# ysymyth/3D-SDN

Hardware: AMD Instinct MI355X
Metric: rendered-objects/sec (FFD decode + transform + silhouette/normal/depth @384, fwd+bwd) (higher is better)
Workload: dtype f32

## Files before the change

### 3d-sdn_amd/csrc/fast_ffd.hip

```cpp
#include "sdn_common.h"

namespace sdn {

constexpr int NCOEF_MAX = 512;

__global__ __launch_bounds__(256) void k_ffd_fwd(const float* __restrict__ Bt, const float* __restrict__ P,
                                                  const int32_t* __restrict__ cls, int vmax, int ncoef,
                                                  float* __restrict__ out)
{
    __shared__ float Ps[3 * NCOEF_MAX];
    const int b = blockIdx.y;
    for (int t = threadIdx.x; t < 3 * ncoef; t += 256) Ps[t] = P[(size_t)b * 3 * ncoef + t];
    __syncthreads();
    const int v = blockIdx.x * 256 + threadIdx.x;
    if (v >= vmax) return;
    const float* bt = Bt + (size_t)cls[b] * ncoef * vmax + v;
    float x = 0.f, y = 0.f, z = 0.f;
#pragma unroll 8
    for (int j = 0; j < ncoef; j++) {
        const float w = bt[(size_t)j * vmax];
        x += Ps[j] * w;
        y += Ps[ncoef + j] * w;
        z += Ps[2 * ncoef + j] * w;
    }
// ... 3 lines not shown
    o[2] = z;
}

constexpr int FFD_BWD_THREADS = 1024, FFD_JB = 4;
__global__ __launch_bounds__(FFD_BWD_THREADS) void k_ffd_bwd(const float* __restrict__ Bt, const int32_t* __restrict__ cls,
                                                              const float* __restrict__ g, int vmax, int ncoef,
                                                              float* __restrict__ grad_P)
{
    constexpr int NW = FFD_BWD_THREADS / 64;
    __shared__ float red[FFD_JB][3][NW];
    const int b = blockIdx.y, j0 = blockIdx.x * FFD_JB;
    const float* bt = Bt + ((size_t)cls[b] * ncoef + j0) * vmax;
    const float* gb = g + (size_t)b * vmax * 3;
    float s[FFD_JB][3];
#pragma unroll
    for (int u = 0; u < FFD_JB; u++) s[u][0] = s[u][1] = s[u][2] = 0.f;
#pragma unroll 2
    for (int v = threadIdx.x; v < vmax; v += FFD_BWD_THREADS) {
        const float g0 = gb[3 * v + 0], g1 = gb[3 * v + 1], g2 = gb[3 * v + 2];
#pragma unroll
        for (int u = 0; u < FFD_JB; u++) {
            const float w = (j0 + u < ncoef) ? bt[(size_t)u * vmax + v] : 0.f;
            s[u][0] += g0 * w;
            s[u][1] += g1 * w;
            s[u][2] += g2 * w;
        }
    }
#pragma unroll
    for (int u = 0; u < FFD_JB; u++) {
#pragma unroll
        for (int o = 32; o > 0; o >>= 1) {
            s[u][0] += __shfl_xor(s[u][0], o, 64);
            s[u][1] += __shfl_xor(s[u][1], o, 64);
            s[u][2] += __shfl_xor(s[u][2], o, 64);
        }
        if ((threadIdx.x & 63) == 0) {
            red[u][0][threadIdx.x >> 6] = s[u][0];
            red[u][1][threadIdx.x >> 6] = s[u][1];
            red[u][2][threadIdx.x >> 6] = s[u][2];
        }
    }
    __syncthreads();
    if (threadIdx.x < 3 * FFD_JB) {
        const int u = threadIdx.x / 3, d = threadIdx.x % 3;
        if (j0 + u < ncoef) {
            float t = 0.f;
#pragma unroll
            for (int w = 0; w < NW; w++) t += red[u][d][w];
            grad_P[((size_t)b * 3 + d) * ncoef + j0 + u] = t;
        }
    }
}

__global__ __launch_bounds__(256) void k_ffd_coefficients(const float* __restrict__ x, const float* __restrict__ M,
                                                          const float* __restrict__ base, int m, int transpose,
                                                          float* __restrict__ out)
{
    extern __shared__ float xrow[];
    float* part = xrow + m;
    const int i = blockIdx.y;
    for (int k = threadIdx.x; k < m; k += 256) xrow[k] = x[(size_t)i * m + k];
    __syncthreads();
    const int jj = threadIdx.x & 63, kq = threadIdx.x >> 6;
    const int j = blockIdx.x * 64 + jj;
    const int per = (m + 3) / 4, k0 = kq * per, k1 = min(m, k0 + per);
    float acc = 0.0f;
    if (j < m) {
        if (transpose) {
            const float* row = M + (size_t)j * m;
#pragma unroll 8
            for (int k = k0; k < k1; k++) acc = fmaf(xrow[k], row[k], acc);
        } else {
#pragma unroll 8
            for (int k = k0; k < k1; k++) acc = fmaf(xrow[k], M[(size_t)k * m + j], acc);
        }
    }
    part[kq * 64 + jj] = acc;
    __syncthreads();
    if (kq == 0 && j < m)
        out[(size_t)i * m + j] = (base ? base[j] : 0.0f) + ((part[jj] + part[64 + jj]) + (part[128 + jj] + part[192 + jj]));
}

}

using namespace sdn;

SDN_API int sdn_ffd_coefficients(const float* x, const float* M, const float* base, int n, int m, int transpose, float* out,
                                 sdnStream stream)
{
    if (!x || !M || !out || n <= 0 || m <= 0 || m > 12288)
        return fail(SDN_EINVAL, "sdn_ffd_coefficients: bad arguments (m <= 12288)");
    hipLaunchKernelGGL(k_ffd_coefficients, dim3(cdiv(m, 64), n), dim3(256), (size_t)(m + 256) * sizeof(float), (hipStream_t)stream,
                       x, M, base, m, transpose, out);
    return check_launch("k_ffd_coefficients");
}

SDN_API int sdn_ffd_decode(const float* Bt, const float* P, const int32_t* cls, int n, int vmax, int ncoef, float* out,
                           sdnStream stream)
{
    if (!Bt || !P || !cls || !out || n <= 0 || vmax <= 0 || ncoef <= 0 || ncoef > NCOEF_MAX)
        return fail(SDN_EINVAL, "sdn_ffd_decode: bad arguments (ncoef <= %d)", NCOEF_MAX);
    hipLaunchKernelGGL(k_ffd_fwd, dim3(cdiv(vmax, 256), n), dim3(256), 0, (hipStream_t)stream, Bt, P, cls, vmax, ncoef,
                       out);
    return check_launch("k_ffd_fwd");
}

SDN_API int sdn_ffd_decode_bwd(const float* Bt, const int32_t* cls, const float* grad_out, int n, int vmax, int ncoef,
                               float* grad_P, sdnStream stream)
{
    if (!Bt || !cls || !grad_out || !grad_P || n <= 0 || vmax <= 0 || ncoef <= 0 || ncoef > NCOEF_MAX)
        return fail(SDN_EINVAL, "sdn_ffd_decode_bwd: bad arguments");
    hipLaunchKernelGGL(k_ffd_bwd, dim3(cdiv(ncoef, FFD_JB), n), dim3(FFD_BWD_THREADS), 0, (hipStream_t)stream, Bt, cls, grad_out, vmax, ncoef,
                       grad_P);
    return check_launch("k_ffd_bwd");
}
```

### 3d-sdn_amd/csrc/raster_bwd.hip

```cpp
#include "raster_math.h"
#include "sdn_common.h"

namespace sdn {

#ifndef SDN_EDGE_CHUNK
#define SDN_EDGE_CHUNK 8
#endif
constexpr int CHUNK = SDN_EDGE_CHUNK;
static_assert(CHUNK == 4 || CHUNK == 8, "k_edge_scan_sil / k_chunk_sum are written for 4 or 8");

struct BwdParams {
    const float* faces;
    const float* textures;
    const float* face_inv;
    const int32_t* face_index_map;
    const float* weight_map;
    const float* depth_map;
    const float* rgb_map;
    const float* g_rgb_out;
    const float* g_alpha_out;
    const float* g_depth_out;
    float* grad_faces;
    float* grad_textures;
    uint32_t* visible;
// ... 187 lines not shown
            if (M.fidx(x, y) != fn) continue;
            float diff_grad = 0.0f;
            if (use_alpha) diff_grad = diff_grad + (1.0f - alpha_out) * M.g_alpha(x, y);
            if (use_rgb) {
#pragma unroll
                for (int k = 0; k < 3; k++) diff_grad = diff_grad + (M.rgb(x, y, k) - rgb_out[k]) * M.g_rgb(x, y, k);
            }
            if (diff_grad <= 0) continue;
            if (nz1) acc0 -= diff_grad / edge_dist(w.p[0][0], w.p[1][0], den1, d1, d1_cross, is_f, P.eps);
            if (nz0) acc1 -= diff_grad / edge_dist(w.p[0][0], w.p[1][0], den0, d1, d1_cross, is_f, P.eps);
        }
    }
}

__global__ __launch_bounds__(256) void k_mark_visible(const int32_t* __restrict__ face_index_map, long npx, int S,
                                                       int nf, uint32_t* __restrict__ visible)
{
    const long i = (long)blockIdx.x * 256 + threadIdx.x;
    if (i >= npx) return;
    const int fn = face_index_map[i];
    if (fn >= 0) visible[(i / ((long)S * S)) * nf + fn] = 1u;
}

__global__ __launch_bounds__(256) void k_hmap(const BwdParams P, float* __restrict__ hmapT)
{
    __shared__ float tile[32][33];
    const int S = P.S, b = blockIdx.z;
    const MapReader M(P, b);
    const int x = blockIdx.x * 32 + (threadIdx.x & 31);
#pragma unroll
    for (int r = 0; r < 4; r++) {
        const int ly = (threadIdx.x >> 5) + 8 * r, y = blockIdx.y * 32 + ly;
        float h = 0.0f;
        if (x < S && y < S) {
            const int fn = M.fidx(x, y);
            if (fn < 0) {
                const float t = (0.0f - 1.0f) * M.g_alpha(x, y);
                h = t > 0.0f ? t : 0.0f;
            } else {
                P.visible[(size_t)b * P.nf + fn] = 1u;
            }
        }
        tile[ly][threadIdx.x & 31] = h;
    }
    __syncthreads();
    const int yt = blockIdx.y * 32 + (threadIdx.x & 31);
#pragma unroll
    for (int r = 0; r < 4; r++) {
        const int lx = (threadIdx.x >> 5) + 8 * r, xt = blockIdx.x * 32 + lx;
        if (xt < S && yt < S) hmapT[((size_t)b * S + xt) * S + yt] = tile[threadIdx.x & 31][lx];
    }
}

__global__ __launch_bounds__(256) void k_compact_rows(const BwdParams P, const float* __restrict__ mapsT,
                                                      size_t rows_per_map, int S, uint16_t* __restrict__ cnt,
                                                      uint16_t* __restrict__ pos, float* __restrict__ val)
{
    const int lane = threadIdx.x & 63;
    const size_t row = (size_t)blockIdx.x * 4 + (threadIdx.x >> 6);
    if (row >= 2 * rows_per_map) return;
    const bool image_row = row < rows_per_map;
    const float* src = mapsT + (image_row ? 0 : row - rows_per_map) * S;
    const int yb = (int)(row / (size_t)S), yy = (int)(row % (size_t)S);
    const MapReader M(P, image_row ? yb : 0);
    auto h_at = [&](const int x) {
        float h = 0.0f;
        if (M.fidx(x, yy) < 0) {
            const float t = (0.0f - 1.0f) * M.g_alpha(x, yy);
            h = t > 0.0f ? t : 0.0f;
        }
        return h;
    };
    uint16_t* c = cnt + row * (S + 1);
    int base = 0;
    for (int x0 = 0; x0 < S; x0 += 128) {
        const int x = x0 + 2 * lane;
        float h0 = 0.0f, h1 = 0.0f;
        if (image_row) {
            if (x < S) h0 = h_at(x);
            if (x + 1 < S) h1 = h_at(x + 1);
        } else if (x + 1 < S && ((S & 1) == 0)) {
            const float2 v = *reinterpret_cast<const float2*>(src + x);
            h0 = v.x;
            h1 = v.y;
        } else {
            if (x < S) h0 = src[x];
            if (x + 1 < S) h1 = src[x + 1];
        }
        const bool nz0 = h0 > 0.0f, nz1 = h1 > 0.0f;
        const unsigned long long m0 = __ballot(nz0), m1 = __ballot(nz1);
        const unsigned long long below = (1ull << lane) - 1ull;
        const int i0 = base + __popcll(m0 & below) + __popcll(m1 & below);
        const int i1 = i0 + (nz0 ? 1 : 0);
        if (x < S) {
            c[x] = (uint16_t)i0;
            if (nz0) {
                pos[row * S + i0] = (uint16_t)x;
                val[row * S + i0] = h0;
            }
        }
        if (x + 1 < S) {
            c[x + 1] = (uint16_t)i1;
            if (nz1) {
                pos[row * S + i1] = (uint16_t)(x + 1);
                val[row * S + i1] = h1;
            }
        }
        base += __popcll(m0) + __popcll(m1);
    }
    if (lane == 0) c[S] = (uint16_t)base;
}

constexpr int PLAN_THREADS = 1024;
__global__ __launch_bounds__(PLAN_THREADS) void k_edge_plan(const BwdParams P)
{
    const long i = (long)blockIdx.x * PLAN_THREADS + threadIdx.x;
    const long total = (long)P.bs * P.nf;
    if (P.sink.grad_verts) {
        const long n = (long)P.bs * P.sink.nv * 3;
        for (long k = i; k < n; k += (long)gridDim.x * PLAN_THREADS) P.sink.grad_verts[k] = 0.0f;
    }
    const int lane = threadIdx.x & 63;
    int from[6], cnt[6];
    uint32_t nchunks = 0;
    bool contributes = false;
    if (i < total) {
        const bool active = (P.flags & (SDN_ALPHA | SDN_RGB)) != 0;
        if (active && P.visible[i] != 0u) {
            float face[9];
#pragma unroll
            for (int k = 0; k < 9; k++) face[k] = P.faces[i * 9 + k];
            if (!is_backface(face)) {
                const float is_f = (float)P.S;
#pragma unroll
                for (int e = 0; e < 6; e++) {
                    const EdgeWalk w = edge_walk(face, e >> 1, e & 1, is_f);
                    from[e] = w.d0_from;
                    cnt[e] = max(w.d0_to - w.d0_from + 1, 0);
                    nchunks += (uint32_t)((cnt[e] + CHUNK - 1) / CHUNK);
                }
                contributes = nchunks != 0;
            }
        }
    }
    __shared__ uint32_t wave_sum[PLAN_THREADS / 64];
    __shared__ uint32_t block_base;
    uint32_t incl = nchunks;
#pragma unroll
    for (int d = 1; d < 64; d <<= 1) {
        const uint32_t o = __shfl_up(incl, d, 64);
        if (lane >= d) incl += o;
    }
    const int wave = threadIdx.x >> 6;
    if (lane == 63) wave_sum[wave] = incl;
    __syncthreads();
    if (threadIdx.x == 0) {
        uint32_t tot = 0;
        for (int w = 0; w < PLAN_THREADS / 64; w++) tot += wave_sum[w];
        block_base = tot ? atomicAdd(P.counter, tot) : 0u;
    }
    __syncthreads();
    uint32_t wave_base = block_base;
    for (int w = 0; w < wave; w++) wave_base += wave_sum[w];
    if (i >= total) return;
    if (!contributes) {
        P.chunk_base[i] = -2;
        return;
    }
    const uint32_t base = wave_base + incl - nchunks;
    if (base + nchunks > P.cap) {
        P.chunk_base[i] = -1;
        for (uint32_t c = base; c < P.cap; c++) P.chunk_desc[c] = make_uint4(0xffffffffu, 0xffffffffu, 0u, 0u);
        return;
    }
    P.chunk_base[i] = (int32_t)base;
    uint32_t c = base;
#pragma unroll
    for (int e = 0; e < 6; e++) {
        for (int s = 0; s < cnt[e]; s += CHUNK)
            P.chunk_desc[c++] = make_uint4((uint32_t)i, (uint32_t)e, (uint32_t)(from[e] + s),
                                           (uint32_t)min(CHUNK, cnt[e] - s));
    }
}

__global__ __launch_bounds__(256) void k_edge_scan(const BwdParams P)
{
    const int lane = threadIdx.x & 63;
    const uint32_t wave = (blockIdx.x * 256u + threadIdx.x) >> 6;
    const uint32_t nwaves = (gridDim.x * 256u) >> 6;
    const uint32_t nchunks = min(*P.counter, P.cap);
    const bool use_alpha = (P.flags & SDN_ALPHA) != 0;
    const bool use_rgb = (P.flags & SDN_RGB) != 0;
    const float is_f = (float)P.S;
    for (uint32_t c = wave; c < nchunks; c += nwaves) {
        const uint4 d = P.chunk_desc[c];
        if (d.x >= (uint32_t)((long)P.bs * P.nf)) {
            if (lane == 0) P.chunk_out[c] = make_float2(0.f, 0.f);
            continue;
        }
        const long i = d.x;
        const int bn = (int)(i / P.nf), fn = (int)(i % P.nf);
        float face[9];
#pragma unroll
        for (int k = 0; k < 9; k++) face[k] = P.faces[i * 9 + k];
        const int axis = (int)(d.y & 1u);
        const EdgeWalk w = edge_walk(face, (int)(d.y >> 1), axis, is_f);
        const MapReader M(P, bn);
        float acc0 = 0.f, acc1 = 0.f;
        for (int s = 0; s < (int)d.w; s++)
            edge_pixel(P, M, w, fn, axis, (int)d.z + s, use_alpha, use_rgb, lane, 64, acc0, acc1);
#pragma unroll
        for (int o = 32; o > 0; o >>= 1) {
            acc0 += __shfl_xor(acc0, o, 64);
            acc1 += __shfl_xor(acc1, o, 64);
        }
        if (lane == 0) P.chunk_out[c] = make_float2(acc0, acc1);
    }
}

#ifndef SDN_LAB_IN_LANE_MAX
#define SDN_LAB_IN_LANE_MAX 32
#endif
constexpr int IN_LANE_MAX = SDN_LAB_IN_LANE_MAX;
#ifndef SDN_LAB_COOP_MAX_WALKS
#define SDN_LAB_COOP_MAX_WALKS 32
#endif
constexpr int COOP_MAX_WALKS = SDN_LAB_COOP_MAX_WALKS;

__global__ __launch_bounds__(256) void k_edge_scan_sil(const BwdParams P)
{
    const int lane = threadIdx.x & 63;
    const uint32_t wave = (blockIdx.x * 256u + threadIdx.x) >> 6;
    const uint32_t nwaves = (gridDim.x * 256u) >> 6;
    const uint32_t nchunks = min(*P.counter, P.cap);
    const int S = P.S;
// ... 507 lines not shown
        return fail(SDN_EINVAL, "rasterize_bwd_core: the vertex sink takes a silhouette-only pass");
    if ((flags & SDN_RGB) && (!rgb_map || !textures))
        return fail(SDN_EINVAL, "sdn_rasterize_bwd: rgb gradients need rgb_map and textures");
    if ((flags & SDN_AA) && (S & 1)) return fail(SDN_EINVAL, "sdn_rasterize_bwd: SDN_AA needs an even internal size");
    size_t off[14], need;
    uint32_t cap;
    bwd_layout(bs, nf, S, off, cap, need);
    if (!workspace || workspace_bytes < need)
        return fail(SDN_ENOMEM, "sdn_rasterize_bwd: workspace %zu < %zu bytes", workspace_bytes, need);
    hipStream_t st = (hipStream_t)stream;
    BwdParams P;
    P.faces = faces;
    P.textures = textures;
    P.face_inv = face_inv;
    P.face_index_map = face_index_map;
    P.weight_map = weight_map;
    P.depth_map = depth_map;
    P.rgb_map = rgb_map;
    P.g_rgb_out = (flags & SDN_RGB) ? g_rgb_out : nullptr;
    P.g_alpha_out = (flags & SDN_ALPHA) ? g_alpha_out : nullptr;
    P.g_depth_out = (flags & SDN_DEPTH) ? g_depth_out : nullptr;
    P.grad_faces = grad_faces;
    P.grad_textures = grad_textures;
    char* ws = (char*)workspace;
    P.counter = (uint32_t*)(ws + off[0]);
    P.visible = (uint32_t*)(ws + off[1]);
    P.chunk_base = (int32_t*)(ws + off[2]);
    P.chunk_desc = (uint4*)(ws + off[3]);
    P.chunk_out = (float2*)(ws + off[4]);
    P.hmap = nullptr;
    P.hmapT = nullptr;
    P.nz_cnt = nullptr;
    P.nz_pos = nullptr;
    P.nz_val = nullptr;
    P.row_cnt = nullptr;
    P.own_rec = nullptr;
    P.own_out = nullptr;
    P.chunk_mask = nullptr;
    P.cap = (flags & SDN_SERIAL_EDGES) ? 0u : cap;
    P.eps = eps;
    P.ts = ts;
    P.bs = bs;
    P.nf = nf;
    P.S = S;
    P.flags = flags;
    P.sink = sink ? *sink : VertexSink{nullptr, 0, 0, 0, 0, nullptr};
    if (!P.g_rgb_out) P.flags &= ~SDN_RGB;
    if (!P.g_alpha_out) P.flags &= ~SDN_ALPHA;
    const long total = (long)bs * nf;
    const long npx = (long)bs * S * S;
    const bool edges = (P.flags & (SDN_ALPHA | SDN_RGB)) != 0;
    if (!edges) P.flags &= ~SDN_SPARSE_GRAD;
    int rc;
    if (edges) {
        hipError_t e = hipMemsetAsync(ws, 0, off[2], st);
        if (e != hipSuccess) return fail(SDN_ELAUNCH, "hipMemsetAsync(plan): %s", hipGetErrorString(e));
        const bool sil_path = (P.flags & SDN_ALPHA) && !(P.flags & SDN_RGB) && !(flags & SDN_SERIAL_EDGES);
        if (!sil_path) {
            hipLaunchKernelGGL(k_mark_visible, dim3(cdiv(npx, 256)), dim3(256), 0, st, face_index_map, npx, S, nf,
                               P.visible);
            if ((rc = check_launch("k_mark_visible"))) return rc;
        }
        if (sil_path) {
            float* hmap = (float*)(ws + off[5]);
            float* hmapT = (float*)(ws + off[6]);
            if (S > 65535) return fail(SDN_EINVAL, "sdn_rasterize_bwd: internal size %d exceeds the 16-bit row index", S);
            uint16_t* cnt = (uint16_t*)(ws + off[7]);
            uint16_t* pos = (uint16_t*)(ws + off[8]);
            float* val = (float*)(ws + off[9]);
            const size_t rows = (size_t)bs * S;
            hipLaunchKernelGGL(k_hmap, dim3(cdiv(S, 32), cdiv(S, 32), bs), dim3(256), 0, st, P, hmapT);
            if ((rc = check_launch("k_hmap"))) return rc;
            hipLaunchKernelGGL(k_compact_rows, dim3((unsigned)cdiv((long)(2 * rows), 4)), dim3(256), 0, st, P, hmapT, rows, S, cnt, pos,
                               val);
            if ((rc = check_launch("k_compact_rows"))) return rc;
            P.hmap = hmap;
            P.hmapT = hmapT;
            P.nz_cnt = cnt;
            P.nz_pos = pos;
            P.nz_val = val;
            if ((size_t)cap * 8 >= (1u << 30)) return fail(SDN_EINVAL, "sdn_rasterize_bwd: %u chunks exceed the 30-bit slot index", cap);
            P.row_cnt = (uint32_t*)(ws + off[10]);
            P.own_rec = (OwnerRec*)(ws + off[11]);
            P.own_out = (float2*)(ws + off[12]);
            P.chunk_mask = (uint8_t*)(ws + off[13]);
        }
    }
    hipLaunchKernelGGL(k_edge_plan, dim3(cdiv(total, PLAN_THREADS)), dim3(PLAN_THREADS), 0, st, P);
    if ((rc = check_launch("k_edge_plan"))) return rc;
    if (edges) {
        {
            TimedLaunch timed(TIME_EDGE_SCAN, st, 0.0);
            if (P.nz_cnt) {
                hipLaunchKernelGGL(k_edge_scan_sil, dim3(256 * 8), dim3(256), 0, st, P);
                const int nrows = 2 * bs * S;
                hipLaunchKernelGGL(k_edge_rows, dim3((unsigned)nrows), dim3(256), (size_t)S * sizeof(float2), st, P, nrows);
                hipLaunchKernelGGL(k_chunk_sum, dim3(cdiv((long)cap, 256)), dim3(256), 0, st, P);
            } else
                hipLaunchKernelGGL(k_edge_scan, dim3(256 * 8), dim3(256), 0, st, P);
        }
        if ((rc = check_launch("k_edge_scan"))) return rc;
    }
    hipLaunchKernelGGL(k_edge_reduce, dim3(cdiv(total, 256)), dim3(256), 0, st, P);
    if ((rc = check_launch("k_edge_reduce"))) return rc;

    const bool need_tex = (P.flags & SDN_RGB) && grad_textures;
    if (need_tex && !(flags & SDN_ACCUMULATE)) {
        const size_t n = (flags & SDN_FACE_COLOR) ? (size_t)total * 3 : (size_t)total * ts * ts * ts * 3;
        hipError_t e = hipMemsetAsync(grad_textures, 0, n * sizeof(float), st);
        if (e != hipSuccess) return fail(SDN_ELAUNCH, "hipMemsetAsync(grad_textures): %s", hipGetErrorString(e));
    }
    if (((P.flags & SDN_DEPTH) && P.g_depth_out) || need_tex) {
        hipLaunchKernelGGL(k_bwd_pixels, dim3(cdiv(npx, 256)), dim3(256), 0, st, P);
        if ((rc = check_launch("k_bwd_pixels"))) return rc;
    }
    return SDN_OK;
}
```

### 3d-sdn_amd/geometric/derender3d/models/transforms.py

```python
import numpy as np
import scipy.special
import torch

from torch.nn.modules import Module


class _Constraint(object):

    class Type:
        symmetry = 0
        homogeneity = 1

    class Axis:
        x = 0
        y = 1
        z = 2

    def __init__(self, type, axis=None, index=None):
        self.type = type
        self.axis = axis
        self.index = index

    @classmethod
    def symmetry(cls, axis):
# ... 1 lines not shown

    @classmethod
    def homogeneity(cls, axis, index):
        return cls(cls.Type.homogeneity, axis=axis, index=list(index))


def apply_constraints(dP, constraints):
    comp = dP.dim() - 4
    for c in constraints:
        ax = comp + 1 + c.axis
        if c.type == _Constraint.Type.symmetry:
            shape = [1] * dP.dim()
            shape[comp] = 3
            sign = torch.tensor([1.0, 1.0, -1.0], dtype=dP.dtype, device=dP.device).reshape(shape)
            dP = (dP + torch.flip(dP, dims=(ax,)) * sign) / 2
        else:
            idx = torch.as_tensor(c.index, device=dP.device)
            planes = dP.index_select(ax, idx)
            total = planes.select(ax, 0)
            for k in range(1, len(c.index)):
                total = total + planes.select(ax, k)
            mean = (total / len(c.index)).unsqueeze(ax).expand_as(planes)
            keep = torch.zeros(3, dtype=torch.bool, device=dP.device)
            keep[c.axis] = True
            shape = [1] * dP.dim()
            shape[comp] = 3
            dP = dP.index_copy(ax, idx, torch.where(keep.reshape(shape), planes, mean))
    return dP


def bernstein_basis(t, one_minus_t, n):
    i = torch.arange(n, dtype=torch.float32)
    binom = torch.tensor(scipy.special.binom(n - 1, np.arange(n)), dtype=torch.float32)
    return binom * torch.pow(t[:, None], i) * torch.pow(one_minus_t[:, None], n - 1 - i)


class FFD(Module):

    Constraint = _Constraint

    @staticmethod
    def flip(x, dim):
        return torch.flip(x, dims=(dim,))

    def __init__(self, vertices, num_grids=4, constraints=None):
        super(FFD, self).__init__()
        if num_grids % 2:
            raise AssertionError('num_grids must be even')
        self.num_grids = num_grids
        self.constraints = list(constraints) if constraints is not None else []
        v = torch.as_tensor(vertices, dtype=torch.float32)
        per_axis = [bernstein_basis(0.5 + v[:, d], 0.5 - v[:, d], num_grids) for d in range(3)]
        B = torch.einsum('ni,nj,nk->nijk', per_axis[0], per_axis[1], per_axis[2])
        lattice = torch.linspace(0, num_grids - 1, num_grids)
        P0 = torch.stack(torch.meshgrid(lattice, lattice, lattice, indexing='ij')) / (num_grids - 1) - 0.5
        self.register_buffer('B', B[:, None], persistent=False)
        self.register_buffer('P0', P0, persistent=False)

    def constrain(self, ffd_coeff):
        g = self.num_grids
        return apply_constraints(ffd_coeff.reshape(3, g, g, g), self.constraints)

    def forward(self, ffd_coeff):
        dP = self.constrain(ffd_coeff)
        n3 = self.num_grids ** 3
        P = (self.P0.to(dP.device) + dP).reshape(3, n3)
        return torch.matmul(self.B.to(dP.device).reshape(-1, n3), P.t())


def constrain_batched(dP, constraints, num_grids):
    return apply_constraints(dP, constraints)


class FFDBank(Module):

    def __init__(self, ffds, faces_list):
        super(FFDBank, self).__init__()
        from sdn_hip import ops
        self.num_grids = ffds[0].num_grids
        self.constraints = ffds[0].constraints
        n3 = self.num_grids ** 3
        self.nverts = [int(f.B.shape[0]) for f in ffds]
        self.nfaces = [int(f.shape[0]) for f in faces_list]
        vmax, fmax = max(self.nverts), max(self.nfaces)
        Bt = torch.zeros(len(ffds), n3, vmax)
        faces = torch.zeros(len(ffds), fmax, 3, dtype=torch.int32)
        for c, (ffd, f) in enumerate(zip(ffds, faces_list)):
            B = ffd.B.reshape(-1, n3)
            Bt[c, :, :B.shape[0]] = B.t()
            Bt[c, :, B.shape[0]:] = B[0][:, None]
            faces[c, :f.shape[0]] = f
        self.register_buffer('Bt', Bt.contiguous(), persistent=False)
        self.register_buffer('faces', faces.contiguous(), persistent=False)
        self.register_buffer('P0', ffds[0].P0.reshape(3, n3).clone(), persistent=False)
        eye = torch.eye(3 * n3).reshape(3 * n3, 3, self.num_grids, self.num_grids, self.num_grids)
        C = constrain_batched(eye, self.constraints, self.num_grids).reshape(3 * n3, 3 * n3)
        self.register_buffer('constraint_matrix', C.contiguous(), persistent=False)

    def decode(self, ffd_coeffs, classes):
        from sdn_hip import ops
        n = ffd_coeffs.shape[0]
        g = self.num_grids
        cls, faces = self._class_rows(classes)
        verts = ops.FFDDecode.apply(ffd_coeffs.reshape(n, 3 * g ** 3), self.Bt, cls, self.constraint_matrix, self.P0)
        return verts, faces

    def _class_rows(self, classes):
        hit = self.__dict__.get('_rows_cache')
        if hit is not None and hit[0] is classes and hit[1] == classes._version:
            return hit[2], hit[3]
        cls = classes.to(torch.int32)
        faces = self.faces.index_select(0, classes.long())
        self.__dict__['_rows_cache'] = (classes, classes._version, cls, faces)
        return cls, faces


    def invalidate_class_cache(self):
        self.__dict__.pop('_rows_cache', None)


class PerspectiveTransform(Module):
    def forward(self,
                vertices,
                scales=None,
                rotations=None,
                translations=None,
                perspective_translations=None,
                zooms=None,
                zoom_tos=None):
        if (vertices.is_cuda and scales is not None and rotations is not None and translations is not None
                and (zoom_tos is None) != (zooms is None) and vertices.dim() == 3):
            from sdn_hip import ops
            n = vertices.shape[0]
            persp = translations if perspective_translations is None else perspective_translations

            def full(x, k):
                return x.reshape(-1, k).expand(n, k) if x.shape[0] != n else x.reshape(n, k)
            t3 = full(translations, 3)
            p3 = t3 if persp is translations else full(persp, 3)
            if zooms is None:
                return ops.PerspectiveTransformFn.apply(vertices, full(scales, 3), full(rotations, 4), t3, p3, full(zoom_tos, 1))
            out, _ = ops.PerspectiveTransformFn.apply(vertices, full(scales, 3), full(rotations, 4), t3, p3, None, full(zooms, 1))
            return out
        return self._forward_elementwise(vertices, scales, rotations, translations, perspective_translations, zooms,
                                         zoom_tos)

    def _forward_elementwise(self, vertices, scales=None, rotations=None, translations=None,
                             perspective_translations=None, zooms=None, zoom_tos=None):
        v = vertices
        if scales is not None:
            v = v * scales[:, None, :]
        if rotations is not None:
            v = torch.matmul(v, quaternion_matrix(rotations).transpose(1, 2))
        if translations is not None:
            v = v + translations[:, None, :]
        centre = translations if perspective_translations is None else perspective_translations
        centre = centre[:, None, :]
# ... 18 lines not shown
```

### 3d-sdn_amd/sdn_hip/ops.py

```python
import ctypes

import numpy as np
import torch
from torch.autograd.function import once_differentiable

from . import (AA, ACCUMULATE, ALPHA, COUNT_WORK, DEPTH, FACE_COLOR, K1_COVERAGE, RGB, SAVE_MAPS, SERIAL_EDGES, STREAM_FACES, check, lib, ptr, raster_bwd_workspace,
               raster_workspace, scene_id_workspace, stream, train_id_workspace, want)

CAMERA_NONE, CAMERA_LOOK, CAMERA_LOOK_AT = 0, 1, 2

import threading

_tls = threading.local()


class verification:

    def __init__(self, serial_edges=None, stream_faces=None, count_work=None):
        new = dict(serial_edges=serial_edges, stream_faces=stream_faces, count_work=count_work)
        self.new = {k: v for k, v in new.items() if v is not None}

    def __enter__(self):
        self.old = {k: getattr(_tls, k, False) for k in self.new}
        for k, v in self.new.items():
# ... 289 lines not shown
        check(lib().sdn_render_maps_bytes(bs, nv, nf0, int(bool(fill_back)), R, flags, ctypes.byref(nstate), ctypes.byref(nbwd),
                                          ctypes.byref(nscr)))
        state = torch.empty(nstate.value, dtype=torch.uint8, device=dev)
        scratch = torch.empty(nscr.value, dtype=torch.uint8, device=dev)
        alpha = torch.empty((bs, R, R), dtype=torch.float32, device=dev)
        normal = torch.empty((bs, 3, R, R), dtype=torch.float32, device=dev) if want_normal else None
        depth = torch.empty((bs, R, R), dtype=torch.float32, device=dev) if want_depth else None
        bg = None
        bg_is_callers = isinstance(background_color, torch.Tensor)
        if want_normal:
            bg = background_color if bg_is_callers else \
                const_f32(background_color if background_color is not None else (0, 0, 0), dev)
            bg = bg.to(device=dev, dtype=torch.float32).contiguous()
            if bg.numel() != 3:
                raise ValueError('render_maps takes one background colour')
        cam = (int(camera_mode), _f32(eye, 'eye'), _f32(direction, 'direction'), _f32(up, 'up'), _f32(width, 'width'),
               int(bool(flip_x)))
        check(lib().sdn_render_maps_fwd(ptr(v), bs, nv, ptr(f), nf0, stride, int(bool(fill_back)), cam[0], ptr(cam[1]),
                                        ptr(cam[2]), ptr(cam[3]), ptr(cam[4]), cam[5], R, flags, float(near), float(far),
                                        float(eps), ptr(bg), ptr(alpha), ptr(normal), ptr(depth), ptr(state), state.numel(),
                                        ptr(scratch), scratch.numel(), stream()))
        if need_grad:
            if bg is not None and bg_is_callers:
                ctx.save_for_backward(v, f, state, cam[1], cam[2], cam[3], cam[4], bg)
                ctx.bg = None
            else:
                ctx.save_for_backward(v, f, state, cam[1], cam[2], cam[3], cam[4])
                ctx.bg = bg
            ctx.cfg = (bs, nv, nf0, stride, int(bool(fill_back)), cam[0], cam[5], R, flags & ~STREAM_FACES, float(eps),
                       float(eps_alpha), nbwd.value, SERIAL_EDGES if _switch('serial_edges') else 0)
        ctx.set_materialize_grads(False)
        return alpha, normal, depth

    @staticmethod
    def backward(ctx, g_alpha, g_normal, g_depth):
        saved = ctx.saved_tensors
        v, f, state, eye, direction, up, width = saved[:7]
        bg = saved[7] if len(saved) > 7 else ctx.bg
        bs, nv, nf0, stride, fill_back, mode, flip_x, R, flags, eps, eps_alpha, nbwd, serial = ctx.cfg
        if g_alpha is None and g_normal is None and g_depth is None:
            return (None,) * 18
        g_alpha = None if g_alpha is None else g_alpha.contiguous()
        g_normal = None if g_normal is None else g_normal.contiguous()
        g_depth = None if g_depth is None else g_depth.contiguous()
        ws = torch.empty(nbwd, dtype=torch.uint8, device=v.device)
        gv = torch.empty_like(v)
        check(lib().sdn_render_maps_bwd(ptr(v), bs, nv, ptr(f), nf0, stride, fill_back, mode, ptr(eye), ptr(direction), ptr(up),
                                        ptr(width), flip_x, R, flags | serial, eps, eps_alpha, ptr(bg), ptr(g_alpha),
                                        ptr(g_normal), ptr(g_depth), ptr(gv), ptr(state), state.numel(), ptr(ws), ws.numel(),
                                        stream()))
        return (gv,) + (None,) * 17


class FFDDecode(torch.autograd.Function):

    @staticmethod
    def forward(ctx, P, Bt, cls, constraint=None, base=None):
        P = _f32(P, 'P')
        Bt = _f32(Bt, 'Bt')
        cls = want(cls, torch.int32, 'cls')
        n = P.shape[0]
        ncoef = Bt.shape[1] if Bt.dim() == 3 else -1
        if constraint is not None:
            Cm = _f32(constraint, 'constraint')
            m = 3 * ncoef
            if P.dim() != 2 or P.shape[1] != m or tuple(Cm.shape) != (m, m) or (base is not None and base.numel() != m):
                raise ValueError('FFDDecode: coefficients [n, 3 ncoef], constraint [3 ncoef, 3 ncoef], base [3, ncoef]')
            base = None if base is None else _f32(base, 'base')
            coeffs = P
            P = torch.empty((n, 3, ncoef), dtype=torch.float32, device=coeffs.device)
            check(lib().sdn_ffd_coefficients(ptr(coeffs), ptr(Cm), ptr(base), n, m, 0, ptr(P), stream()))
        else:
            Cm = None
        if P.dim() != 3 or P.shape[1] != 3 or Bt.dim() != 3 or P.shape[2] != ncoef or cls.numel() != n:
            raise ValueError('FFDDecode: P [n,3,ncoef], Bt [classes,ncoef,vmax], cls [n]')
        vmax = Bt.shape[2]
        out = torch.empty((n, vmax, 3), dtype=torch.float32, device=P.device)
        check(lib().sdn_ffd_decode(ptr(Bt), ptr(P), ptr(cls), n, vmax, ncoef, ptr(out), stream()))
        if Cm is None:
            ctx.save_for_backward(Bt, cls)
        else:
            ctx.save_for_backward(Bt, cls, Cm)
        ctx.cfg = (n, vmax, ncoef)
        return out

    @staticmethod
    def backward(ctx, g):
        Bt, cls = ctx.saved_tensors[:2]
        n, vmax, ncoef = ctx.cfg
        g = g.contiguous()
        gP = torch.empty((n, 3, ncoef), dtype=torch.float32, device=g.device)
        check(lib().sdn_ffd_decode_bwd(ptr(Bt), ptr(cls), ptr(g), n, vmax, ncoef, ptr(gP), stream()))
        if len(ctx.saved_tensors) == 3:
            gc = torch.empty((n, 3 * ncoef), dtype=torch.float32, device=g.device)
            check(lib().sdn_ffd_coefficients(ptr(gP), ptr(ctx.saved_tensors[2]), None, n, 3 * ncoef, 1, ptr(gc), stream()))
            return gc, None, None, None, None
        return gP, None, None, None, None


class PoseParamsFn(torch.autograd.Function):

    @staticmethod
    def forward(ctx, theta, log_scales):
        th = _f32(theta, 'theta').reshape(-1)
        n = th.shape[0]
        ls = _f32(log_scales, 'log_scales').reshape(n, 3)
        quat = torch.empty(n, 4, dtype=torch.float32, device=th.device)
        scales = torch.empty(n, 3, dtype=torch.float32, device=th.device)
        check(lib().sdn_pose_params(ptr(th), ptr(ls), n, ptr(quat), ptr(scales), stream()))
        ctx.save_for_backward(th, scales)
        ctx.shapes = (theta.shape, log_scales.shape)
        ctx.set_materialize_grads(False)
        return quat, scales

    @staticmethod
    def backward(ctx, g_quat, g_scales):
        th, scales = ctx.saved_tensors
        n = th.shape[0]
        want_t, want_s = ctx.needs_input_grad
        if g_quat is None and g_scales is None:
            return None, None
        gq = g_quat.contiguous() if g_quat is not None else None
        gs = g_scales.contiguous() if g_scales is not None else None
        gt = torch.empty(n, dtype=torch.float32, device=th.device) if want_t else None
        gl = torch.empty(n, 3, dtype=torch.float32, device=th.device) if want_s else None
        if gt is None and gl is None:
            return None, None
        check(lib().sdn_pose_params_bwd(ptr(th), ptr(scales), ptr(gq), ptr(gs), n, ptr(gt), ptr(gl), stream()))
        return (gt.reshape(ctx.shapes[0]) if gt is not None else None, gl.reshape(ctx.shapes[1]) if gl is not None else None)


class PoseAlgebraFn(torch.autograd.Function):

    @staticmethod
    def forward(ctx, centre, extent, focals, theta_deltas, log_scales, log_depths, translation2ds, training, image_size,
                render_size):
        c = _f32(centre, 'centre')
        n = c.shape[0]
        c = c.reshape(n, 2)
        e = _f32(extent, 'extent').reshape(n, 2)
        f = _f32(focals, 'focals').reshape(n)
        d = _f32(theta_deltas, 'theta_deltas').reshape(n, 2)
        ls = _f32(log_scales, 'log_scales').reshape(n, 3)
        ld = _f32(log_depths, 'log_depths').reshape(n)
        t2 = _f32(translation2ds, 'translation2ds').reshape(n, 2)
        dev = c.device
        new = lambda *shape: torch.empty(shape, dtype=torch.float32, device=dev)
        thetas, alphas, rot, scales, depths = new(n, 1), new(n, 1), new(n, 4), new(n, 3), new(n, 1)
        c2, trans, persp, zooms = new(n, 2), new(n, 3), new(n, 3), new(n, 1)
        check(lib().sdn_pose_algebra(ptr(c), ptr(e), ptr(f), ptr(d), ptr(ls), ptr(ld), ptr(t2), n, int(bool(training)),
# ... 1080 lines not shown
```

### include/sdn_hip.h

```cpp
#ifndef SDN_HIP_H
#define SDN_HIP_H

#include <stddef.h>
#include <stdint.h>

#ifdef __cplusplus
extern "C" {
#endif

typedef void* sdnStream;

#define SDN_OK 0
#define SDN_EINVAL (-1)
#define SDN_ELAUNCH (-2)
#define SDN_ENOMEM (-3)

#define SDN_RGB 1
#define SDN_ALPHA 2
#define SDN_DEPTH 4
#define SDN_AA 8
#define SDN_FACE_COLOR 16
#define SDN_SAVE_MAPS 32
#define SDN_ACCUMULATE 64
#define SDN_STREAM_FACES 256
// ... 6 lines not shown
const char* sdn_last_error(void);
#define SDN_ABI_VERSION 20
int sdn_version(void);

int sdn_project_vertices(const float* verts, int bs, int nv, int camera_mode, const float* eye,
                         const float* dir, const float* up, const float* width, int flip_x,
                         float* out, sdnStream stream);
int sdn_project_vertices_bwd(const float* verts, int bs, int nv, int camera_mode, const float* eye,
                             const float* dir, const float* up, const float* width, int flip_x,
                             const float* grad_out, float* grad_verts, sdnStream stream);

int sdn_gather_faces(const float* verts, const int32_t* faces_idx, int bs, int nv, int nf0,
                     long faces_batch_stride, int fill_back, float* faces_out, sdnStream stream);
int sdn_gather_faces_bwd(const float* grad_faces, const int32_t* faces_idx, int bs, int nv, int nf0,
                         long faces_batch_stride, int fill_back, float* grad_verts, sdnStream stream);

int sdn_face_normals(const float* faces, long n_faces_total, float* normals, sdnStream stream);
int sdn_face_normals_bwd(const float* faces, const float* grad_normals, long n_faces_total,
                         float* grad_faces, sdnStream stream);

int sdn_raster_workspace_bytes(int bs, int nf, int S, size_t* out);

int sdn_rasterize_fwd(const float* faces, const float* textures, int ts, int bs, int nf, int S,
                      double near, double far, double eps, const float* bg, int bg_per_batch, int flags,
                      float* face_inv, int32_t* face_index_map, float* weight_map, float* depth_map,
                      float* rgb_map, float* rgb_out, float* alpha_out, float* depth_out,
                      void* workspace, size_t workspace_bytes, sdnStream stream);

int sdn_raster_work_counters(const void* workspace, int bs, int nf, int S, unsigned long long* out3, sdnStream stream);

int sdn_raster_phase_clocks(const void* workspace, int bs, int nf, int S, unsigned long long* out8, sdnStream stream);

int sdn_raster_bwd_workspace_bytes(int bs, int nf, int S, size_t* out);
int sdn_rasterize_bwd(const float* faces, const float* textures, int ts, int bs, int nf, int S,
                      double eps, int flags, const float* face_inv, const int32_t* face_index_map,
                      const float* weight_map, const float* depth_map, const float* rgb_map,
                      const float* g_rgb_out, const float* g_alpha_out, const float* g_depth_out,
                      float* grad_faces, float* grad_textures, void* workspace, size_t workspace_bytes,
                      sdnStream stream);

int sdn_render_maps_bytes(int bs, int nv, int nf0, int fill_back, int image_size, int flags, size_t* state_bytes,
                          size_t* bwd_workspace_bytes, size_t* fwd_scratch_bytes);
int sdn_render_maps_fwd(const float* verts, int bs, int nv, const int32_t* faces_idx, int nf0, long faces_batch_stride,
                        int fill_back, int camera_mode, const float* eye, const float* dir, const float* up,
                        const float* width, int flip_x, int image_size, int flags, double near, double far, double eps,
                        const float* bg, float* alpha_out, float* normal_out, float* depth_out, void* state,
                        size_t state_bytes, void* scratch, size_t scratch_bytes, sdnStream stream);
int sdn_render_maps_bwd(const float* verts, int bs, int nv, const int32_t* faces_idx, int nf0, long faces_batch_stride,
                        int fill_back, int camera_mode, const float* eye, const float* dir, const float* up,
                        const float* width, int flip_x, int image_size, int flags, double eps, double eps_alpha,
                        const float* bg, const float* g_alpha, const float* g_normal, const float* g_depth, float* grad_verts,
                        const void* state, size_t state_bytes, void* workspace, size_t workspace_bytes, sdnStream stream);

int sdn_ffd_decode(const float* Bt, const float* P, const int32_t* cls, int n, int vmax, int ncoef,
                   float* out, sdnStream stream);
int sdn_ffd_decode_bwd(const float* Bt, const int32_t* cls, const float* grad_out, int n, int vmax,
                       int ncoef, float* grad_P, sdnStream stream);
int sdn_ffd_coefficients(const float* x, const float* M, const float* base, int n, int m, int transpose, float* out,
                         sdnStream stream);


#define SDN_STAT_SLOTS 8
int sdn_conv_gemm_workspace_bytes(int N, int OH, int OW, int Cop, size_t* out);
int sdn_conv_gemm(const float* in, int N, int IH, int IW, int Cip, float* out, int OH, int OW, int Cop, int QH, int QW,
                  int istride, int ostride, int py, int px, int ntaps, const int8_t* dy, const int8_t* dx, int pad_mode,
                  int in_relu, const void* w_packed, int Kp, int w_rows, const float* bias, int act,
                  double* stats, int accumulate, int precision, void* workspace, size_t workspace_bytes,
                  sdnStream stream);

int sdn_conv_gemm_phases(const float* in, int N, int IH, int IW, int Cip, float* out, int OH, int OW, int Cop, int istride,
                         int ostride, int nphase, const int32_t* QH, const int32_t* QW, const int32_t* py, const int32_t* px,
                         const int32_t* ntaps, const int8_t* taps, int pad_mode, int in_relu, const void* const* w_packed,
                         const int32_t* Kp, int w_rows, const float* bias, int act, double* stats, int accumulate,
                         int precision, sdnStream stream);

int sdn_conv_wgrad(const float* rows, const float* gath, float* dw, int N, int QH, int QW, int Cr, int GH, int GW, int Cc,
                   int istride, int ntaps, const int8_t* dy, const int8_t* dx, int pad_mode, int relu_rows,
                   int relu_gath, int splits, int precision, void* workspace, size_t workspace_bytes, sdnStream stream);
int sdn_conv_wgrad_narrow(const float* rows, const float* gath, float* dw, int N, int QH, int QW, int Cr, int rows_used,
                          int GH, int GW, int Cc, int ntaps, const int8_t* dy, const int8_t* dx, int pad_mode,
                          int relu_rows, int relu_gath, sdnStream stream);

int sdn_conv_wgrad_head_mfma(const float* rows, const float* gath, float* dw, int N, int QH, int QW, int Cr, int rows_used,
                             int GH, int GW, int Cc, int ntaps, const int8_t* dy, const int8_t* dx, int pad_mode,
                             int relu_rows, int relu_gath, sdnStream stream);

int sdn_conv_narrow_fwd(const float* in, int N, int IH, int IW, int Cip, float* out, int QH, int QW, int Cop,
                        int rows_used, const float* w_dense, int KH, int KW, int dy_min, int dx_min, int pad_mode,
                        int in_relu, const float* bias, int act, sdnStream stream);

int sdn_conv_head_steps(int Cip, int KH, int KW, int* steps);
int sdn_conv_head_mfma(const float* in, int N, int IH, int IW, int Cip, float* out, int QH, int QW, int Cop, int rows_used,
                       const void* w_frag, int KH, int KW, int dy_min, int dx_min, int pad_mode, int in_relu,
                       const float* bias, int act, double* stats, sdnStream stream);

int sdn_in_apply(float* z, const double* stats, float* mr, const float* res, float* out2, int N, int HW, int C, int Cp,
                 float eps, int act, int res_relu, float momentum, float* running_mean, float* running_var, void* planes,
                 long plane_stride, int planes_relu, sdnStream stream);
#define SDN_IN_BWD_SUMS_ZEROED 8
int sdn_in_bwd(float* g, const float* stored, const float* mr, double* sums, int N, int HW, int Cp, int mode, void* planes,
               long plane_stride, sdnStream stream);
int sdn_act_bwd(float* g, const float* y, float* bias_grad, long npos, int Cp, int act, void* planes, long plane_stride,
                sdnStream stream);
int sdn_reflect_fold(const float* gp, float* out, int N, int H, int W, int Cp, int pad, int accumulate, sdnStream stream);
int sdn_conv_pack_weights(const float* w, int R, int C, long sr, long sc, const int32_t* tapidx, int ntaps, int Ccp,
                          int Kp, int rows, void* packed, sdnStream stream);
// ... 227 lines not shown
```

Before: 22950.

## Decode FFD from separable per-axis Bernstein factors and fuse edge plan with row compaction

Adds a forward FFD decode kernel that reads 12 per-axis Bernstein factors per vertex and forms the 64 tensor-product weights in registers, instead of streaming the full 64-row basis matrix. The factors are precomputed on the host at construction and used only when their outer product exactly reproduces Bt. This cuts forward memory traffic at the cost of extra multiplies. Separately, the backward rasterizer's edge-plan and row-compaction launches are merged into one kernel with block-range dispatch, removing one launch.

```diff
diff --git a/3d-sdn_amd/csrc/fast_ffd.hip b/3d-sdn_amd/csrc/fast_ffd.hip
--- a/3d-sdn_amd/csrc/fast_ffd.hip
+++ b/3d-sdn_amd/csrc/fast_ffd.hip
@@ -79,6 +79,42 @@
     }
 }
 
+constexpr int FFD_G = 4, FFD_NC = FFD_G * FFD_G * FFD_G;
+
+__global__ __launch_bounds__(256) void k_ffd_fwd_factored(const float* __restrict__ fac, const float* __restrict__ P,
+                                                           const int32_t* __restrict__ cls, int vmax, float* __restrict__ out)
+{
+    __shared__ float Ps[3 * FFD_NC];
+    const int b = blockIdx.y;
+    if (threadIdx.x < 3 * FFD_NC) Ps[threadIdx.x] = P[(size_t)b * 3 * FFD_NC + threadIdx.x];
+    __syncthreads();
+    const int v = blockIdx.x * 256 + threadIdx.x;
+    if (v >= vmax) return;
+    const float* f = fac + (size_t)cls[b] * 3 * FFD_G * vmax + v;
+    float bx[FFD_G], by[FFD_G], bz[FFD_G], t[FFD_G * FFD_G];
+#pragma unroll
+    for (int i = 0; i < FFD_G; i++) {
+        bx[i] = f[(size_t)i * vmax];
+        by[i] = f[(size_t)(FFD_G + i) * vmax];
+        bz[i] = f[(size_t)(2 * FFD_G + i) * vmax];
+    }
+#pragma unroll
+    for (int i = 0; i < FFD_G * FFD_G; i++) t[i] = bx[i / FFD_G] * by[i % FFD_G];
+    float x = 0.f, y = 0.f, z = 0.f;
+#pragma unroll
+    for (int j = 0; j < FFD_NC; j++) {
+        const float w = t[j / FFD_G] * bz[j % FFD_G];
+        x += Ps[j] * w;
+        y += Ps[FFD_NC + j] * w;
+        z += Ps[2 * FFD_NC + j] * w;
+    }
+    float* o = out + ((size_t)b * vmax + v) * 3;
+    o[0] = x;
+    o[1] = y;
+    o[2] = z;
+}
+
+
 __global__ __launch_bounds__(256) void k_ffd_coefficients(const float* __restrict__ x, const float* __restrict__ M,
                                                           const float* __restrict__ base, int m, int transpose,
                                                           float* __restrict__ out)
@@ -125,6 +161,11 @@
 SDN_API int sdn_ffd_decode(const float* Bt, const float* P, const int32_t* cls, int n, int vmax, int ncoef, float* out,
                            sdnStream stream)
 {
+    if (ncoef == (FFD_NC | SDN_FFD_FACTORS)) {
+        if (!Bt || !P || !cls || !out || n <= 0 || vmax <= 0) return fail(SDN_EINVAL, "sdn_ffd_decode: bad arguments (factors)");
+        hipLaunchKernelGGL(k_ffd_fwd_factored, dim3(cdiv(vmax, 256), n), dim3(256), 0, (hipStream_t)stream, Bt, P, cls, vmax, out);
+        return check_launch("k_ffd_fwd_factored");
+    }
     if (!Bt || !P || !cls || !out || n <= 0 || vmax <= 0 || ncoef <= 0 || ncoef > NCOEF_MAX)
         return fail(SDN_EINVAL, "sdn_ffd_decode: bad arguments (ncoef <= %d)", NCOEF_MAX);
     hipLaunchKernelGGL(k_ffd_fwd, dim3(cdiv(vmax, 256), n), dim3(256), 0, (hipStream_t)stream, Bt, P, cls, vmax, ncoef,
diff --git a/3d-sdn_amd/csrc/raster_bwd.hip b/3d-sdn_amd/csrc/raster_bwd.hip
--- a/3d-sdn_amd/csrc/raster_bwd.hip
+++ b/3d-sdn_amd/csrc/raster_bwd.hip
@@ -263,12 +263,10 @@
     }
 }
 
-__global__ __launch_bounds__(256) void k_compact_rows(const BwdParams P, const float* __restrict__ mapsT,
-                                                      size_t rows_per_map, int S, uint16_t* __restrict__ cnt,
-                                                      uint16_t* __restrict__ pos, float* __restrict__ val)
-{
-    const int lane = threadIdx.x & 63;
-    const size_t row = (size_t)blockIdx.x * 4 + (threadIdx.x >> 6);
+__device__ __forceinline__ void compact_row(const BwdParams& P, const float* __restrict__ mapsT, size_t rows_per_map, int S,
+                                            uint16_t* __restrict__ cnt, uint16_t* __restrict__ pos, float* __restrict__ val,
+                                            const size_t row, const int lane)
+{
     if (row >= 2 * rows_per_map) return;
     const bool image_row = row < rows_per_map;
     const float* src = mapsT + (image_row ? 0 : row - rows_per_map) * S;
@@ -323,13 +321,13 @@
 }
 
 constexpr int PLAN_THREADS = 1024;
-__global__ __launch_bounds__(PLAN_THREADS) void k_edge_plan(const BwdParams P)
-{
-    const long i = (long)blockIdx.x * PLAN_THREADS + threadIdx.x;
+__device__ __forceinline__ void edge_plan_block(const BwdParams& P, const unsigned block, const unsigned nblocks)
+{
+    const long i = (long)block * PLAN_THREADS + threadIdx.x;
     const long total = (long)P.bs * P.nf;
     if (P.sink.grad_verts) {
         const long n = (long)P.bs * P.sink.nv * 3;
-        for (long k = i; k < n; k += (long)gridDim.x * PLAN_THREADS) P.sink.grad_verts[k] = 0.0f;
+        for (long k = i; k < n; k += (long)nblocks * PLAN_THREADS) P.sink.grad_verts[k] = 0.0f;
     }
     const int lane = threadIdx.x & 63;
     int from[6], cnt[6];
@@ -392,6 +390,21 @@
             P.chunk_desc[c++] = make_uint4((uint32_t)i, (uint32_t)e, (uint32_t)(from[e] + s),
                                            (uint32_t)min(CHUNK, cnt[e] - s));
     }
+}
+
+__global__ __launch_bounds__(PLAN_THREADS) void k_edge_plan(const BwdParams P) { edge_plan_block(P, blockIdx.x, gridDim.x); }
+
+__global__ __launch_bounds__(PLAN_THREADS) void k_plan_rows(const BwdParams P, const unsigned plan_blocks,
+                                                             const float* __restrict__ mapsT, size_t rows_per_map, int S,
+                                                             uint16_t* __restrict__ cnt, uint16_t* __restrict__ pos,
+                                                             float* __restrict__ val)
+{
+    if (blockIdx.x < plan_blocks) {
+        edge_plan_block(P, blockIdx.x, plan_blocks);
+        return;
+    }
+    const size_t row = (size_t)(blockIdx.x - plan_blocks) * (PLAN_THREADS / 64) + (threadIdx.x >> 6);
+    compact_row(P, mapsT, rows_per_map, S, cnt, pos, val, row, threadIdx.x & 63);
 }
 
 __global__ __launch_bounds__(256) void k_edge_scan(const BwdParams P)
@@ -1005,6 +1018,7 @@
     const bool edges = (P.flags & (SDN_ALPHA | SDN_RGB)) != 0;
     if (!edges) P.flags &= ~SDN_SPARSE_GRAD;
     int rc;
+    bool planned = false;
     if (edges) {
         hipError_t e = hipMemsetAsync(ws, 0, off[2], st);
         if (e != hipSuccess) return fail(SDN_ELAUNCH, "hipMemsetAsync(plan): %s", hipGetErrorString(e));
@@ -1024,9 +1038,11 @@
             const size_t rows = (size_t)bs * S;
             hipLaunchKernelGGL(k_hmap, dim3(cdiv(S, 32), cdiv(S, 32), bs), dim3(256), 0, st, P, hmapT);
             if ((rc = check_launch("k_hmap"))) return rc;
-            hipLaunchKernelGGL(k_compact_rows, dim3((unsigned)cdiv((long)(2 * rows), 4)), dim3(256), 0, st, P, hmapT, rows, S, cnt, pos,
-                               val);
-            if ((rc = check_launch("k_compact_rows"))) return rc;
+            const unsigned plan_blocks = cdiv(total, PLAN_THREADS);
+            hipLaunchKernelGGL(k_plan_rows, dim3(plan_blocks + cdiv((long)(2 * rows), PLAN_THREADS / 64)), dim3(PLAN_THREADS), 0, st, P,
+                               plan_blocks, hmapT, rows, S, cnt, pos, val);
+            if ((rc = check_launch("k_plan_rows"))) return rc;
+            planned = true;
             P.hmap = hmap;
             P.hmapT = hmapT;
             P.nz_cnt = cnt;
@@ -1039,8 +1055,10 @@
             P.chunk_mask = (uint8_t*)(ws + off[13]);
         }
     }
-    hipLaunchKernelGGL(k_edge_plan, dim3(cdiv(total, PLAN_THREADS)), dim3(PLAN_THREADS), 0, st, P);
-    if ((rc = check_launch("k_edge_plan"))) return rc;
+    if (!planned) {
+        hipLaunchKernelGGL(k_edge_plan, dim3(cdiv(total, PLAN_THREADS)), dim3(PLAN_THREADS), 0, st, P);
+        if ((rc = check_launch("k_edge_plan"))) return rc;
+    }
     if (edges) {
         {
             TimedLaunch timed(TIME_EDGE_SCAN, st, 0.0);
diff --git a/3d-sdn_amd/geometric/derender3d/models/transforms.py b/3d-sdn_amd/geometric/derender3d/models/transforms.py
--- a/3d-sdn_amd/geometric/derender3d/models/transforms.py
+++ b/3d-sdn_amd/geometric/derender3d/models/transforms.py
@@ -77,6 +77,7 @@
         v = torch.as_tensor(vertices, dtype=torch.float32)
         per_axis = [bernstein_basis(0.5 + v[:, d], 0.5 - v[:, d], num_grids) for d in range(3)]
         B = torch.einsum('ni,nj,nk->nijk', per_axis[0], per_axis[1], per_axis[2])
+        self.per_axis = torch.stack(per_axis)
         lattice = torch.linspace(0, num_grids - 1, num_grids)
         P0 = torch.stack(torch.meshgrid(lattice, lattice, lattice, indexing='ij')) / (num_grids - 1) - 0.5
         self.register_buffer('B', B[:, None], persistent=False)
@@ -116,18 +117,32 @@
             Bt[c, :, B.shape[0]:] = B[0][:, None]
             faces[c, :f.shape[0]] = f
         self.register_buffer('Bt', Bt.contiguous(), persistent=False)
+        self.register_buffer('factors', self._factors(ffds, Bt), persistent=False)
         self.register_buffer('faces', faces.contiguous(), persistent=False)
         self.register_buffer('P0', ffds[0].P0.reshape(3, n3).clone(), persistent=False)
         eye = torch.eye(3 * n3).reshape(3 * n3, 3, self.num_grids, self.num_grids, self.num_grids)
         C = constrain_batched(eye, self.constraints, self.num_grids).reshape(3 * n3, 3 * n3)
         self.register_buffer('constraint_matrix', C.contiguous(), persistent=False)
 
+    def _factors(self, ffds, Bt):
+        g = self.num_grids
+        if g != 4 or any(getattr(f, 'per_axis', None) is None for f in ffds):
+            return None
+        fac = torch.zeros(len(ffds), 3, g, Bt.shape[2])
+        for c, ffd in enumerate(ffds):
+            pa = ffd.per_axis.to(torch.float32).cpu().transpose(1, 2)
+            fac[c, :, :, :pa.shape[2]] = pa
+            fac[c, :, :, pa.shape[2]:] = pa[:, :, :1]
+        prod = ((fac[:, 0, :, None, None, :] * fac[:, 1, None, :, None, :]) * fac[:, 2, None, None, :, :]).reshape(Bt.shape)
+        return fac.contiguous() if torch.equal(prod, Bt.cpu()) else None
+
     def decode(self, ffd_coeffs, classes):
         from sdn_hip import ops
         n = ffd_coeffs.shape[0]
         g = self.num_grids
         cls, faces = self._class_rows(classes)
-        verts = ops.FFDDecode.apply(ffd_coeffs.reshape(n, 3 * g ** 3), self.Bt, cls, self.constraint_matrix, self.P0)
+        verts = ops.FFDDecode.apply(ffd_coeffs.reshape(n, 3 * g ** 3), self.Bt, cls, self.constraint_matrix, self.P0,
+                                    self.factors)
         return verts, faces
 
     def _class_rows(self, classes):
diff --git a/3d-sdn_amd/sdn_hip/ops.py b/3d-sdn_amd/sdn_hip/ops.py
--- a/3d-sdn_amd/sdn_hip/ops.py
+++ b/3d-sdn_amd/sdn_hip/ops.py
@@ -365,10 +365,13 @@
         return (gv,) + (None,) * 17
 
 
+FFD_FACTORS = 0x10000
+
+
 class FFDDecode(torch.autograd.Function):
 
     @staticmethod
-    def forward(ctx, P, Bt, cls, constraint=None, base=None):
+    def forward(ctx, P, Bt, cls, constraint=None, base=None, factors=None):
         P = _f32(P, 'P')
         Bt = _f32(Bt, 'Bt')
         cls = want(cls, torch.int32, 'cls')
@@ -389,7 +392,13 @@
             raise ValueError('FFDDecode: P [n,3,ncoef], Bt [classes,ncoef,vmax], cls [n]')
         vmax = Bt.shape[2]
         out = torch.empty((n, vmax, 3), dtype=torch.float32, device=P.device)
-        check(lib().sdn_ffd_decode(ptr(Bt), ptr(P), ptr(cls), n, vmax, ncoef, ptr(out), stream()))
+        if factors is not None:
+            factors = _f32(factors, 'factors')
+            if ncoef != 64 or tuple(factors.shape) != (Bt.shape[0], 3, 4, vmax):
+                raise ValueError('FFDDecode: factors [classes, 3, 4, vmax] go with Bt [classes, 64, vmax]')
+            check(lib().sdn_ffd_decode(ptr(factors), ptr(P), ptr(cls), n, vmax, ncoef | FFD_FACTORS, ptr(out), stream()))
+        else:
+            check(lib().sdn_ffd_decode(ptr(Bt), ptr(P), ptr(cls), n, vmax, ncoef, ptr(out), stream()))
         if Cm is None:
             ctx.save_for_backward(Bt, cls)
         else:
@@ -407,8 +416,8 @@
         if len(ctx.saved_tensors) == 3:
             gc = torch.empty((n, 3 * ncoef), dtype=torch.float32, device=g.device)
             check(lib().sdn_ffd_coefficients(ptr(gP), ptr(ctx.saved_tensors[2]), None, n, 3 * ncoef, 1, ptr(gc), stream()))
-            return gc, None, None, None, None
-        return gP, None, None, None, None
+            return gc, None, None, None, None, None
+        return gP, None, None, None, None, None
 
 
 class PoseParamsFn(torch.autograd.Function):
diff --git a/include/sdn_hip.h b/include/sdn_hip.h
--- a/include/sdn_hip.h
+++ b/include/sdn_hip.h
@@ -82,6 +82,7 @@
                         const float* bg, const float* g_alpha, const float* g_normal, const float* g_depth, float* grad_verts,
                         const void* state, size_t state_bytes, void* workspace, size_t workspace_bytes, sdnStream stream);
 
+#define SDN_FFD_FACTORS 0x10000
 int sdn_ffd_decode(const float* Bt, const float* P, const int32_t* cls, int n, int vmax, int ncoef,
                    float* out, sdnStream stream);
 int sdn_ffd_decode_bwd(const float* Bt, const int32_t* cls, const float* grad_out, int n, int vmax,
```

New measurement: 22900. Within noise of the previous version (-0.2%).
